# danavery/audio-tokens

Hardware: AMD Instinct MI355X
Metric: STFT frames/sec through K-means+tokenize, n_mels=64 vocab=8192 (higher is better)
Workload: dtype f32; 1 GPU; configs[3] per-GPU shard x1: 22500+2500 clips/GPU of 10 s @22.05 kHz (43075000 frames/GPU), n_mels=64, vocab_size=8192, niter=20, k-means batches of 10000 files on a 2097152-row subsample; parallelism=dp1

## Files before the change

audio_tokens_amd/_lib.py:

```python
from __future__ import annotations

import ctypes
from pathlib import Path

_PKG = Path(__file__).resolve().parent
LIB_PATH = _PKG / "libaudio_tokens_amd.so"

AT_LAYOUT_MEL_MAJOR = 0
AT_LAYOUT_FRAME_MAJOR = 1

_c = ctypes
_vp, _i32, _i64 = _c.c_void_p, _c.c_int, _c.c_int64

class PrunedArgs(_c.Structure):
    _fields_ = [("x", _vp), ("n", _i64), ("d", _i32), ("c", _vp), ("k", _i32), ("order", _vp), ("hint_sorted", _vp),
                ("cperm", _vp), ("ng", _i32), ("bounds", _vp), ("guess_only", _i32), ("use_filter", _i32),
                ("prepass_done", _i32), ("image_current", _i32), ("ids", _vp), ("dist_or_null", _vp)]


class FlacInfo(_c.Structure):
    _fields_ = [("channels", _c.c_int32), ("bits_per_sample", _c.c_int32), ("sample_rate", _c.c_int32),
                ("min_block", _c.c_int32), ("max_block", _c.c_int32), ("variable_blocksize", _c.c_int32),
                ("total_samples", _i64)]

# ... 25 lines not shown
    "at_workspace_bytes": (_i64, [_vp]),
    "at_background_stream": (_i32, [_vp, _c.POINTER(_vp)]),
    "at_debug_set": (_i32, [_vp, _c.c_char_p, _i32]),
    "at_debug_get": (_i32, [_vp, _c.c_char_p, _c.POINTER(_i32)]),
    "at_diag_errors": (_i32, [_c.POINTER(_i64), _c.POINTER(_i32), _c.POINTER(_i64), _c.POINTER(_i32), _c.c_char_p, _i32, _i32]),
    "at_debug_leave_error_pending": (_i32, []),
    "at_rand_perm_mt19937": (_i32, [_i64, _i64, _vp]),
    "at_rand_perm_prefix_mt19937": (_i32, [_i64, _i64, _i64, _vp]),
    "at_rand_perm_prefix_device": (_i32, [_vp, _i64, _i64, _i64, _vp, _vp]),
    "at_mel_filterbank_host": (_i32, [_i32, _i32, _i32, _vp]),
    "at_num_frames": (_i64, [_i64, _i32]),
    "at_split_clusters_host": (_i32, [_i32, _i32, _i64, _vp, _vp, _c.POINTER(_i32)]),
    "at_logmel_f32": (_i32, [_vp, _vp, _i64, _i64, _i64, _i32, _i32, _i32, _i32, _vp, _vp, _i32, _i32, _vp]),
    "at_resample_length": (_i64, [_i64, _i32, _i32]),
    "at_resample_taps_host": (_i32, [_i32, _i32, _c.POINTER(_i32), _c.POINTER(_i32), _c.POINTER(_i32), _vp, _i64]),
    "at_resample_f32": (_i32, [_vp, _vp, _i64, _i64, _i64, _i32, _i32, _vp, _i64, _vp]),
    "at_minmax_scale_clips_f32": (_i32, [_vp, _vp, _i64, _i64, _vp]),
    "at_conv1d_mel_f32": (_i32, [_vp, _vp, _i64, _i32, _vp, _vp, _i32, _i32, _i32, _vp, _vp]),
    "at_logmel_minmax_f32": (_i32, [_vp, _vp, _i64, _i64, _i64, _i32, _i32, _i32, _i32, _vp, _vp, _i32, _vp]),
    "at_l2norm_rows_f32": (_i32, [_vp, _vp, _i64, _i32, _vp, _vp]),
    "at_assign_f32": (_i32, [_vp, _vp, _i64, _i32, _vp, _i32, _vp, _vp, _vp]),
    "at_assign_hinted_f32": (_i32, [_vp, _vp, _i64, _i32, _vp, _i32, _vp, _vp, _vp, _vp, _vp, _vp]),
    "at_group_rows_kd_host": (_i32, [_vp, _i32, _i32, _i32, _vp]),
    "at_group_min_dist_f32": (_i32, [_vp, _vp, _i32, _i32, _vp, _i32, _vp, _vp]),
    "at_visit_order_f32": (_i32, [_vp, _vp, _vp, _i64, _i32, _vp, _vp, _vp]),
    "at_prune_stats": (_i32, [_vp, _c.POINTER(_i64), _c.POINTER(_i64), _i32]),
    "at_assign_coarse_f32": (_i32, [_vp, _vp, _i64, _i32, _vp, _i32, _vp, _i32, _vp, _vp, _vp, _vp, _vp]),
    "at_filter_stats": (_i32, [_vp, _c.POINTER(_i64), _c.POINTER(_i64), _c.POINTER(_c.c_double), _c.POINTER(_i64),
                               _c.POINTER(_i64), _c.POINTER(_i64), _i32]),
    "at_filter_probe_f32": (_i32, [_vp, _vp, _i64, _i32, _vp, _i32, _vp, _vp, _vp, _i32, _vp, _vp, _vp,
                                   _c.POINTER(_i64), _vp]),
    "at_group_means_f32": (_i32, [_vp, _vp, _i32, _i32, _vp, _i32, _vp, _vp]),
    "at_group_neighbours_f32": (_i32, [_vp, _vp, _i32, _i32, _i32, _vp, _vp]),
    "at_assign_pruned_f32": (_i32, [_vp, _vp, _vp]),
    "at_prune_mask_f32": (_i32, [_vp, _vp, _i64, _i32, _vp, _i32, _vp, _vp, _i32, _vp, _i32, _vp]),
    "at_gather_rows_f32": (_i32, [_vp, _vp, _i32, _vp, _i64, _vp, _vp]),
    "at_centroid_accum_f32": (_i32, [_vp, _vp, _i64, _i32, _vp, _i32, _vp, _vp, _vp, _vp, _vp]),
    "at_centroid_finalize_f32": (_i32, [_vp, _vp, _i64, _vp, _i64, _i32, _i32, _i32, _vp, _vp, _vp]),
    "at_split_clusters_f32": (_i32, [_vp, _i32, _i32, _i64, _vp, _vp, _vp, _vp]),
    "at_lloyd_stats_f64": (_i32, [_vp, _vp, _i32, _vp, _i64, _i32, _vp, _vp]),
    "at_comm_allgather_f32": (_i32, [_vp, _vp, _vp, _vp, _i64, _vp]),
    "at_comm_allreduce_ordered_f32": (_i32, [_vp, _vp, _vp, _vp, _vp, _i64, _vp]),
    "at_lloyd_stats_split_f32": (_i32, [_vp, _i32, _i32, _i64, _vp, _vp, _vp, _vp, _i64, _i32, _vp, _vp]),
    "at_sum_parts_f32": (_i32, [_vp, _vp, _i64, _i32, _i64, _vp, _vp]),
    "at_sum_f32": (_i32, [_vp, _vp, _i64, _vp, _vp]),
    "at_any_nonfinite_f32": (_i32, [_vp, _vp, _i64, _vp, _vp]),
    "at_logmel_nonfinite_take": (_i32, [_vp, _vp, _vp]),
    "at_centroid_accum_defer": (_i32, [_vp, _i32]),
    "at_centroid_accum_join": (_i32, [_vp, _vp]),
    "at_token_histogram_i64": (_i32, [_vp, _vp, _i64, _i32, _vp, _vp]),
    "at_token_stats_f64": (_i32, [_vp, _vp, _i32, _vp, _vp, _vp, _vp]),
    "at_silhouette_f32": (_i32, [_vp, _vp, _i32, _vp, _i64, _vp, _vp, _vp, _vp]),
    "at_average_precision_f32": (_i32, [_vp, _vp, _i64, _vp, _i64, _i64, _i32, _vp, _vp, _vp, _vp, _vp]),
    "at_ranking_metrics_f32": (_i32, [_vp, _vp, _i64, _vp, _i64, _i64, _i32, _vp, _vp, _vp, _vp, _vp, _vp, _vp, _vp]),
    "at_threshold_counts_f32": (_i32, [_vp, _vp, _i64, _vp, _i64, _i64, _i32, _c.c_float, _vp, _vp, _vp]),
    "at_knn_f32": (_i32, [_vp, _vp, _i64, _i32, _vp, _i32, _i32, _vp, _vp, _vp]),
    "at_assign_ip_f32": (_i32, [_vp, _vp, _i64, _i32, _vp, _i32, _vp, _vp, _vp]),
    "at_renorm_rows_f32": (_i32, [_vp, _vp, _i64, _i32, _vp]),
    "at_pq_encode_f32": (_i32, [_vp, _vp, _i64, _i32, _i32, _i32, _vp, _vp, _vp, _vp, _vp]),
    "at_pq_decode_f32": (_i32, [_vp, _vp, _i64, _i32, _i32, _i32, _vp, _vp, _vp]),
    "at_flac_index_host": (_i32, [_vp, _i64, _c.POINTER(FlacInfo), _vp, _i64, _c.POINTER(_i64)]),
    "at_flac_decode_f32": (_i32, [_vp, _i64, _vp, _i64, _i32, _vp, _i64, _vp, _vp, _vp]),
# ... 79 lines not shown
```

audio_tokens_amd/backend.py:

```python
from __future__ import annotations

import ctypes
import os

import numpy as np
import torch

from . import _lib

_vp = ctypes.c_void_p


def _ptr(t) -> _vp:
    return _vp(t.data_ptr()) if t is not None else _vp(None)


def _np_ptr(a: np.ndarray) -> _vp:
    return _vp(a.ctypes.data)


class HostHelpers:

    def __init__(self):
        self.lib = _lib.load()
# ... 107 lines not shown
        return int(ns.value)


class HipBackend(HostHelpers):
    def __init__(self, device=None):
        super().__init__()
        if not torch.cuda.is_available():
            raise RuntimeError("audio_tokens_amd: no ROCm device visible (torch.cuda.is_available() "
                               "is False) and there is no CPU fallback")
        if device is None:
            device = torch.device("cuda", torch.cuda.current_device())
        device = torch.device(device)
        if device.type != "cuda":
            raise RuntimeError(f"audio_tokens_amd: device must be a ROCm GPU, got {device}")
        if device.index is None:
            device = torch.device("cuda", torch.cuda.current_device())
        self.device = device
        self.ctx = _lib.context(device.index)
        self.assign_trace = None
        self.assign_trace_only = None
        self.frontend_calls = 0
        self.frontend_bytes = 0
        self.switches = {"filter": os.environ.get("AT_FILTER", "1") != "0",
                         "c2f_fused": os.environ.get("AT_C2F_FUSED", "1") != "0"}

    def debug_set(self, name: str, value: int) -> None:
        _lib.check(self.lib.at_debug_set(self.ctx.handle, name.encode(), int(value)))

    def debug_get(self, name: str) -> int:
        v = ctypes.c_int(0)
        _lib.check(self.lib.at_debug_get(self.ctx.handle, name.encode(), ctypes.byref(v)))
        return int(v.value)

    def diag_errors(self, reset=False) -> dict:
        stale, tol = ctypes.c_int64(0), ctypes.c_int64(0)
        sc, tc = ctypes.c_int(0), ctypes.c_int(0)
        where = ctypes.create_string_buffer(512)
        _lib.check(self.lib.at_diag_errors(ctypes.byref(stale), ctypes.byref(sc), ctypes.byref(tol), ctypes.byref(tc),
                                           where, 512, 1 if reset else 0))
        return {"stale_seen": int(stale.value), "stale_last_code": int(sc.value), "tolerated": int(tol.value),
                "tolerated_last_code": int(tc.value), "where": where.value.decode()}

    def _stream(self) -> _vp:
        return _vp(torch.cuda.current_stream(self.device).cuda_stream)

    def _f32(self, t, name="tensor") -> torch.Tensor:
        if isinstance(t, np.ndarray):
# ... 405 lines not shown
        if rec is not None:
            e0, e1 = torch.cuda.Event(enable_timing=True), torch.cuda.Event(enable_timing=True)
            e0.record(torch.cuda.current_stream(self.device))
        with torch.cuda.device(self.device):
            _lib.check(self.lib.at_assign_hinted_f32(self.ctx.handle, _ptr(x), n, d, _ptr(c), k, _ptr(hint_ids),
                                                     _ptr(order), _ptr(hint_sorted), _ptr(ids), _ptr(dist),
                                                     self._stream()))
        if rec is not None:
            e1.record(torch.cuda.current_stream(self.device))
            rec.append(("hinted", n, d, k, e0, e1))
        return ids, dist

    def group_min_dist(self, c, cperm) -> torch.Tensor:
        c = self._f32(c)
        k, d = c.shape
        assert cperm.dtype == torch.int32 and cperm.is_contiguous() and cperm.numel() % 32 == 0
        ng = cperm.numel() // 32
        dmin = self.empty((k, ng))
        with torch.cuda.device(self.device):
            _lib.check(self.lib.at_group_min_dist_f32(self.ctx.handle, _ptr(c), k, d, _ptr(cperm), ng, _ptr(dmin),
                                                      self._stream()))
        return dmin

    def visit_order(self, ids, dis, k):
        n = ids.numel()
        assert ids.dtype == torch.int64 and ids.is_contiguous()
        order, hs = self.empty((n,), torch.int32), self.empty((n,), torch.int32)
        with torch.cuda.device(self.device):
            _lib.check(self.lib.at_visit_order_f32(self.ctx.handle, _ptr(ids), _ptr(dis), n, k, _ptr(order), _ptr(hs),
                                                   self._stream()))
        return order, hs

    def visit_order_beside(self, ids, dis, k, sum_out=None):
        main = torch.cuda.current_stream(self.device)
        side = getattr(self, "_order_stream", None)
        if side is None:
            side = self._order_stream = torch.cuda.Stream(self.device)
        side.wait_stream(main)
        with torch.cuda.stream(side):
            if sum_out is not None:
                self.sum_f64(dis, out=sum_out)
                sum_out.record_stream(side)
            out = self.visit_order(ids, dis, k)

        def join(out=out, ids=ids, dis=dis):
            torch.cuda.current_stream(self.device).wait_stream(side)
# ... 199 lines not shown

    def centroid_finalize(self, parts, k, d):
        if parts.dim() == 1:
            parts = parts.unsqueeze(0)
        assert parts.is_contiguous() and parts.shape[1] >= k * d + k
        n_parts = parts.shape[0]
        cent = self.empty((k, d))
        hassign = self.empty((k,))
        stride = parts.stride(0)
        with torch.cuda.device(self.device):
            _lib.check(self.lib.at_centroid_finalize_f32(
                self.ctx.handle, _ptr(parts), stride, _vp(parts.data_ptr() + 4 * k * d), stride, n_parts,
                k, d, _ptr(cent), _ptr(hassign), self._stream()))
        return cent, hassign

    def split_clusters_device(self, hassign, cent, n: int, nsplit_out) -> None:
        k, d = cent.shape
        assert hassign.dtype == torch.float32 and cent.dtype == torch.float32 and nsplit_out.dtype == torch.int32
        assert hassign.is_contiguous() and cent.is_contiguous() and hassign.numel() == k
        with torch.cuda.device(self.device):
            _lib.check(self.lib.at_split_clusters_f32(self.ctx.handle, d, k, n, _ptr(hassign), _ptr(cent), _ptr(nsplit_out),
                                                      self._stream()))

    def _objective_parts(self, parts, k, d, objs):
        if objs is not None:
            assert objs.dtype == torch.float64 and objs.is_contiguous()
            return _ptr(objs), 1, objs.numel()
        if parts.dim() == 1:
            parts = parts.unsqueeze(0)
        off, total = self.part_layout(k, d)
        assert parts.is_contiguous() and parts.shape[1] == total
        return _vp(parts.data_ptr() + 4 * off), total // 2, parts.shape[0]

    def lloyd_stats(self, hassign, parts, k: int, d: int, stats_row, objs=None) -> None:
        assert stats_row.dtype == torch.float64
        ptr, stride, n_parts = self._objective_parts(parts, k, d, objs)
        with torch.cuda.device(self.device):
            _lib.check(self.lib.at_lloyd_stats_f64(self.ctx.handle, _ptr(hassign), k, ptr, stride, n_parts, _ptr(stats_row),
                                                   self._stream()))

    def lloyd_stats_split(self, hassign, cent, n: int, nsplit_out, parts, stats_row, objs=None) -> None:
        k, d = cent.shape
        assert stats_row.dtype == torch.float64 and nsplit_out.dtype == torch.int32
        assert hassign.dtype == torch.float32 and cent.dtype == torch.float32
        assert hassign.is_contiguous() and cent.is_contiguous() and hassign.numel() == k
        ptr, stride, n_parts = self._objective_parts(parts, k, d, objs)
# ... 144 lines not shown
```

audio_tokens_amd/csrc/lloyd.hip:

```cpp
#include <climits>

#include "at_internal.h"
#include "mt19937_dev.h"

namespace {

constexpr int WG = 256;
constexpr long SPLIT_CYCLES = 64;
constexpr int SPLIT_BLOCKS = 16;
constexpr int SPLIT_ROUND = SPLIT_BLOCKS * WG;

__device__ __forceinline__ float rand_float_of(uint32_t raw) { return __uint2float_rn(raw) * 2.3283064365386963e-10f; }

__device__ void lloyd_stats_block(const float* __restrict__ hassign, int k, const double* obj_parts, long obj_stride,
                                  int n_parts, double* __restrict__ stats) {
    __shared__ double s1[WG / 64], s2[WG / 64];
    const int t = threadIdx.x;
    double a = 0.0, b = 0.0;
    for (int c = t; c < k; c += WG) {
        const double h = (double)hassign[c];
        a += h;
        b += h * h;
    }
    for (int off = 32; off > 0; off >>= 1) {
        a += __shfl_down(a, off);
        b += __shfl_down(b, off);
    }
    if ((t & 63) == 0) { s1[t >> 6] = a; s2[t >> 6] = b; }
    __syncthreads();
    if (t == 0) {
        double tot = 0.0, sq = 0.0;
        for (int w = 0; w < WG / 64; w++) { tot += s1[w]; sq += s2[w]; }
        double obj = 0.0;
        for (int p = 0; p < n_parts; p++) obj += obj_parts[(size_t)p * obj_stride];
        stats[0] = obj;
        stats[1] = sq * k / (tot * tot);
    }
    __syncthreads();
}

__global__ __launch_bounds__(WG) void lloyd_stats_kernel(const float* __restrict__ hassign, int k, const double* obj_parts,
                                                        long obj_stride, int n_parts, double* __restrict__ stats) {
    lloyd_stats_block(hassign, k, obj_parts, obj_stride, n_parts, stats);
}

__global__ __launch_bounds__(WG) void split_clusters_kernel(int d, int k, long n, float* hassign, float* cent,
                                                           int* __restrict__ empties, int* __restrict__ nsplit_out,
                                                           const uint32_t* __restrict__ raw, long raw_n,
                                                           const uint32_t* __restrict__ state_end, int p_lds,
                                                           const double* obj_parts, long obj_stride, int n_parts,
                                                           double* __restrict__ stats) {
    extern __shared__ float pl[];
    __shared__ at_mt::State mt;
    __shared__ float draws[at_mt::N];
    __shared__ int wave_val[4][WG / 64];
    __shared__ int n_empty;
    const int t = threadIdx.x, lane = t & 63, wave = t >> 6;

    if (stats) lloyd_stats_block(hassign, k, obj_parts, obj_stride, n_parts, stats);
    {
        bool any = false;
        for (int c = t; c < k; c += WG) any |= hassign[c] == 0.0f;
        if (!__syncthreads_or(any)) {
            if (t == 0) *nsplit_out = 0;
            return;
        }
    }
    if (t == 0) n_empty = 0;
    __syncthreads();
    for (int base = 0; base < k; base += WG) {
        const int c = base + t;
        const bool e = c < k && hassign[c] == 0.0f;
        const unsigned long long b = __ballot(e);
        if (lane == 0) wave_val[0][wave] = __popcll(b);
        __syncthreads();
        int off = n_empty;
        for (int w = 0; w < wave; w++) off += wave_val[0][w];
        if (e) empties[off + __popcll(b & ((1ull << lane) - 1ull))] = c;
        __syncthreads();
        if (t == 0) n_empty += wave_val[0][0] + wave_val[0][1] + wave_val[0][2] + wave_val[0][3];
        __syncthreads();
    }
    const int ne = n_empty;
    if (ne == 0) {
        if (t == 0) *nsplit_out = 0;
        return;
    }

    const double denom = (double)(float)(n - k);
    auto prob = [&](int c) { return (float)(((double)hassign[c] - 1.0) / denom); };
    if (p_lds) {
        for (int c = t; c < k; c += WG) pl[c] = prob(c);
        __syncthreads();
    }
    const double up = 1.0 + 1.0 / 1024.0, down = 1.0 - 1.0 / 1024.0;
    long pos = 0;
    int cur = 0, win = 0, wlen = 0;
    bool own = false;
    int done = 0;
    for (int e = 0; e < ne; e++) {
        const int ci = empties[e];
        int cj0 = 0, donor = -1;
        long left = SPLIT_CYCLES * k + 1024;
        while (left > 0 && donor < 0) {
            if (pos + SPLIT_ROUND <= raw_n) {
                uint32_t draw[SPLIT_BLOCKS];
#pragma unroll
                for (int i = 0; i < SPLIT_BLOCKS; i++) draw[i] = raw[pos + i * WG + t];
                int mine = INT_MAX;
#pragma unroll
                for (int i = 0; i < SPLIT_BLOCKS; i++) {
                    const int j = i * WG + t;
                    int cj = cj0 + j;
                    cj -= (cj / k) * k;
                    const float pc = p_lds ? pl[cj] : prob(cj);
                    const bool acc = rand_float_of(draw[i]) < pc;
                    const unsigned long long b = __ballot(acc);
                    if (b && mine == INT_MAX) mine = i * WG + wave * 64 + (__ffsll((long long)b) - 1);
                }
                if (lane == 0) wave_val[0][wave] = mine;
                __syncthreads();
                int first = INT_MAX;
#pragma unroll
                for (int w = 0; w < WG / 64; w++) first = min(first, wave_val[0][w]);
                __syncthreads();
                if (first != INT_MAX) {
                    donor = (int)((cj0 + (long)first) % k);
                    pos += first + 1;
                } else {
                    pos += SPLIT_ROUND;
                    left -= SPLIT_ROUND;
                    cj0 = (int)((cj0 + (long)SPLIT_ROUND) % k);
                }
                continue;
            }
            if (win == wlen) {
                if (pos < raw_n) {
                    wlen = (int)min((long)at_mt::N, raw_n - pos);
                    for (int q = t; q < wlen; q += WG) draws[q] = rand_float_of(raw[pos + q]);
                } else {
                    wlen = at_mt::N;
                    if (!own) {
                        for (int q = t; q < at_mt::N; q += WG) mt.st[0][q] = state_end[q];
                        __syncthreads();
                        own = true;
                        cur = 0;
                    }
                    const uint32_t* nw = at_mt::regenerate(mt, cur);
// ... 8 lines not shown
            if (t < chunk) {
                const int cj = (cj0 + t) % k;
                acc = draws[win + t] < (p_lds ? pl[cj] : prob(cj));
            }
            const unsigned long long b = __ballot(acc);
            if (lane == 0) wave_val[0][wave] = b ? wave * 64 + (__ffsll((long long)b) - 1) : INT_MAX;
            __syncthreads();
            const int first = min(min(wave_val[0][0], wave_val[0][1]), min(wave_val[0][2], wave_val[0][3]));
            __syncthreads();
            if (first < chunk) {
                donor = (cj0 + first) % k;
                win += first + 1;
                pos += first + 1;
            } else {
                win += chunk;
                pos += chunk;
                left -= chunk;
                cj0 = (cj0 + chunk) % k;
            }
        }
        if (donor < 0) break;
        float* dst = cent + (size_t)ci * d;
        float* src = cent + (size_t)donor * d;
        for (int j = t; j < d; j += WG) {
            const double a = (double)src[j];
            dst[j] = (float)(a * ((j & 1) ? down : up));
            src[j] = (float)(a * ((j & 1) ? up : down));
        }
        if (t == 0) {
            const float half = hassign[donor] / 2;
            hassign[ci] = half;
            hassign[donor] -= half;
        }
        done++;
        __syncthreads();
        if (p_lds && t == 0) {
            pl[ci] = prob(ci);
            pl[donor] = prob(donor);
        }
        __syncthreads();
    }
    if (t == 0) *nsplit_out = done == ne ? ne : -1;
}

}

extern "C" {

int at_split_clusters_f32(at_ctx* ctx, int d, int k, int64_t n, float* hassign, float* centroids, int32_t* nsplit_out,
                          void* stream_) {
    return at_lloyd_stats_split_f32(ctx, d, k, n, hassign, centroids, nsplit_out, nullptr, 0, 0, nullptr, stream_);
}

int at_lloyd_stats_split_f32(at_ctx* ctx, int d, int k, int64_t n, float* hassign, float* centroids, int32_t* nsplit_out,
                             const double* obj_parts, int64_t obj_part_stride, int n_parts, double* stats, void* stream_) {
    AT_REQUIRE(ctx && hassign && centroids && nsplit_out && d > 0 && k > 0 && n >= k, "at_split_clusters_f32: bad arguments");
    AT_REQUIRE(!stats || (obj_parts && n_parts >= 1 && (reinterpret_cast<uintptr_t>(obj_parts) & 7u) == 0 &&
                          (reinterpret_cast<uintptr_t>(stats) & 7u) == 0),
               "at_lloyd_stats_split_f32: obj_parts / stats must be given together, 8-byte aligned");
    hipStream_t stream = static_cast<hipStream_t>(stream_);
    AT_HIP(hipSetDevice(ctx->device));
    int* empties = static_cast<int*>(at_ws(ctx, WS_SPLIT_LIST, (size_t)k * sizeof(int), stream));
    if (!empties) return AT_E_NOMEM;
    const uint32_t *raw = nullptr, *state_end = nullptr;
    int64_t raw_n = 0;
    int rc = at_mt_cached_draws(ctx, 1234u, stream, &raw, &raw_n, &state_end);
    if (rc) return rc;
    const int p_lds = k <= 16384;
    const size_t lds = p_lds ? (size_t)k * sizeof(float) : 0;
    AT_RAISE_LDS(ctx, split_clusters_kernel, lds);
    AT_LAUNCH(split_clusters_kernel, dim3(1), dim3(WG), lds, stream, d, k, (long)n, hassign, centroids, empties,
                       nsplit_out, raw, (long)raw_n, state_end, p_lds, obj_parts, (long)obj_part_stride, n_parts, stats);
    return AT_OK;
}

int at_lloyd_stats_f64(at_ctx* ctx, const float* hassign, int k, const double* obj_parts, int64_t obj_part_stride,
                       int n_parts, double* stats, void* stream_) {
    AT_REQUIRE(ctx && hassign && obj_parts && stats && k > 0 && n_parts >= 1, "at_lloyd_stats_f64: bad arguments");
    AT_REQUIRE((reinterpret_cast<uintptr_t>(obj_parts) & 7u) == 0 && (reinterpret_cast<uintptr_t>(stats) & 7u) == 0,
               "at_lloyd_stats_f64: obj_parts / stats must be 8-byte aligned");
    hipStream_t stream = static_cast<hipStream_t>(stream_);
    AT_HIP(hipSetDevice(ctx->device));
    AT_LAUNCH(lloyd_stats_kernel, dim3(1), dim3(WG), 0, stream, hassign, k, obj_parts, (long)obj_part_stride,
                       n_parts, stats);
    return AT_OK;
}

}
```

audio_tokens_amd/ops.py:

```python
from __future__ import annotations

import collections
import math
import os
import statistics
import sys
import time
from collections import OrderedDict

import numpy as np
import torch

from .backend import default_backend

__all__ = ["LogMelSpectrogram", "Resample", "Kmeans", "IndexFlatL2", "IndexFlatIP", "normalize_rows", "silhouette_samples",
           "silhouette_score", "average_precision", "mean_average_precision", "roc_auc", "mean_roc_auc",
           "roc_auc_score", "d_prime", "f1_score", "hamming_loss", "classification_metrics", "load_flac",
           "load_flac_batch", "AudioTokenizer", "ProductQuantizer"]


def _is_host(x) -> bool:
    return isinstance(x, np.ndarray) or (isinstance(x, torch.Tensor) and x.device.type == "cpu")


# ... 267 lines not shown

        niter = self.niter
        stats_dev = be.zeros((max(niter, 1), 2), torch.float64)
        nsplit_dev = be.zeros((max(niter, 1),), torch.int32)
        obj_off, part_len = be.part_layout(k, d)
        scatter_exchange = dist.on and (self.exchange == "scatter" or (self.exchange == "auto" and part_len * 4 > (4 << 20)))
        t0 = time.time()
        prof = self.phase_seconds

        def lap(name, t_prev):
            if prof is None:
                return t_prev
            be.synchronize()
            now = time.perf_counter()
            prof[name] = prof.get(name, 0.0) + (now - t_prev)
            return now

        prune = (self.prune and not spherical and hasattr(be, "assign_pruned") and d in (64, 128) and k >= 1024
                 and (k + 31) // 32 <= 512 and xs.shape[0] >= 4096)
        ids = dis = order = vorder = None
        member_order = prune and xs.shape[0] < 96 * k
        regrouping = None
        regrouping_is_late = False

        def regroup_beside(c):
            h, ready = be.to_host_async(c)

            def job():
                ready.synchronize()
                return be.group_rows_kd(h.numpy())
            return _grouper().submit(job)

        if prune:
            upload = getattr(be, "from_host_async", be.from_host)
            cached = getattr(self, "_cperm_cache", None)
            if init_centroids is not None and cached is not None and cached[0] == (k, d):
                cperm = cached[1]
                if not (init_centroids is getattr(self, "centroids_device", None)
                        or init_centroids is self.__dict__.get("_centroids_host")):
                    regrouping = regroup_beside(cent)
            else:
                cperm = be.from_host(be.group_rows_kd(be.to_host(cent)))
            gnbr = None
        late_regroup = niter - 6 if niter >= 10 else -1
        paced = collections.deque()
        iter_ms = None
        last_done = None
        timed_events = hasattr(be, "record_event_timed")

        def late_due(it):
            if late_regroup < 0 or it < niter // 2:
                return False
            return it >= late_regroup or (iter_ms is not None and (niter - it) * iter_ms <= 4.5)

        def pruned_assign(it):
            nonlocal cperm, regrouping, regrouping_is_late, gnbr
            if regrouping is not None and regrouping.done():
                cperm = upload(regrouping.result())
                regrouping = None
            elif (it == 2 and init_centroids is None and regrouping is None) or (late_due(it) and not regrouping_is_late):
                regrouping_is_late = late_due(it)
                regrouping = regroup_beside(cent)
            dmin = be.group_min_dist(cent, cperm)
            if ids is None:
                gnbr = be.group_neighbours(be.group_means(cent, cperm), 8)
                return be.assign_c2f(xs, cent, cperm, dmin, gnbr)
            return be.assign_pruned(xs, cent, vorder if vorder is not None else be.visit_order(ids, dis, k),
                                    cperm, dmin, image_current=True)

        for it in range(niter):
            tp = time.perf_counter()
            if prune:
                ids, dis = pruned_assign(it)
            elif spherical:
                ids, dis = be.assign_ip(xs, cent)
            elif ids is None:
                ids, dis = be.assign(xs, cent)
            else:
                ids, dis = be.assign_hinted(xs, cent, ids, order)
            tp = lap("assign", tp)
            part = be.empty((part_len,))
            obj_view = part[obj_off:obj_off + 2].view(torch.float64)
            beside = prune and not member_order and self.order_beside and it + 1 < niter
            sjoin = None
            if not beside:
# ... 30 lines not shown
            if hasattr(be, "lloyd_stats_split"):
                be.lloyd_stats_split(hassign, cent, ns, nsplit_dev[it:it + 1], parts, stats_dev[it], objs=objs)
            else:
                be.lloyd_stats(hassign, parts, k, d, stats_dev[it], objs=objs)
                be.split_clusters_device(hassign, cent, ns, nsplit_dev[it:it + 1])
            if spherical:
                cent = be.renorm_rows(cent)
            tp = lap("exchange+finalize+split", tp)
            if prune and timed_events:
                paced.append(be.record_event_timed())
                if len(paced) > 3:
                    done = paced.popleft()
                    done.synchronize()
                    if last_done is not None:
                        iter_ms = last_done.elapsed_time(done)
                    last_done = done
        self._last_assign = ids
        self._stats_pending = (stats_dev[:niter], nsplit_dev[:niter], t0)
        if self.verbose:
            for it, st in enumerate(self.iteration_stats):
                print(f"  Iteration {it} ({st['time']:.2f} s, search {st['time_search']:.2f} s): "
                      f"objective={st['obj']:g} imbalance={st['imbalance_factor']:.3f} nsplit={st['nsplit']}", flush=True)
        if prune:
            if regrouping is not None and (regrouping.done() or regrouping_is_late):
                cperm = upload(regrouping.result())
            self._cperm_cache = ((k, d), cperm)
            self._grouping_of_result = cperm
        return self._finish(cent, sync)

    def _subsample_perm(self, n, m):
        key = (int(n), self.seed, int(m))
        cache = self.__dict__.setdefault("_perm_cache", OrderedDict())
        hit = cache.get(key)
        if hit is None:
            hit = cache[key] = self.backend.rand_perm_prefix_device(n, self.seed, m)
            while len(cache) > 2:
                cache.popitem(last=False)
        return hit

    def _read_stats(self, stats_dev, nsplit_dev, t0):
        be = self.backend
        st, ns = be.to_host(stats_dev), be.to_host(nsplit_dev)
        if (ns < 0).any():
            raise RuntimeError("Kmeans: split_clusters found no donor (every cluster has at most one point)")
        el = time.time() - t0
        return [dict(obj=float(np.float32(st[i, 0])), time=el * (i + 1) / len(ns), time_search=el * (i + 1) / len(ns),
                     imbalance_factor=float(st[i, 1]), nsplit=int(ns[i])) for i in range(len(ns))]

    @property
    def iteration_stats(self):
        if self._stats_pending is not None:
            self._iteration_stats = self._read_stats(*self._stats_pending)
            self._stats_pending = None
        return self._iteration_stats

    @property
    def obj(self):
        return np.array([s["obj"] for s in self.iteration_stats], dtype=np.float32)

    @property
    def centroids(self):
        if self._centroids_host is None and self.centroids_device is not None:
            self._centroids_host = self.backend.to_host(self.centroids_device)
        return self._centroids_host

    def lend_grouping(self, table) -> None:
        cached = getattr(self, "_cperm_cache", None)
        be = self.backend
        if cached is not None and hasattr(be, "remember_grouping"):
            table = be.to_host(table) if isinstance(table, torch.Tensor) else np.asarray(table)
            if table.shape == cached[0]:
                be.remember_grouping(table, cached[1])

    def _finish(self, cent, sync=True):
        self.centroids_device = cent
        self._centroids_host = None
        self.index = (IndexFlatIP if self.spherical else IndexFlatL2)(self.d, backend=self.backend)
        self.index.add(cent)
        be = self.backend
        if getattr(self, "_grouping_of_result", None) is not None and hasattr(be, "remember_grouping"):
            if sync:
                be.remember_grouping(self.centroids, self._grouping_of_result)
            self._grouping_of_result = None
        if not sync:
            return None
        st = self.iteration_stats
        return float(st[-1]["obj"]) if st else 0.0


_GROUPER = None


def _grouper():
    global _GROUPER
    if _GROUPER is None:
        from concurrent.futures import ThreadPoolExecutor
        _GROUPER = ThreadPoolExecutor(max_workers=1, thread_name_prefix="at-grouping")
    return _GROUPER


class IndexFlatL2:

    def __init__(self, d, backend=None):
        self.d = int(d)
        self.backend = backend or default_backend()
        self._c = None
        self._prune = None
        self.prune = True
        self.rows_coherent = True

    @property
    def ntotal(self) -> int:
        return 0 if self._c is None else int(self._c.shape[0])

    def reset(self) -> None:
        self._c = None
        self._prune = None

    def add(self, c) -> None:
        c = self.backend._f32(c)
        assert c.dim() == 2 and c.shape[1] == self.d, f"expected [n, {self.d}]"
        self._c = c.clone() if self._c is None else torch.cat([self._c, c], 0)
        self._prune = None

    def assign(self, x, want_dist=True):
        be = self.backend
        c = self._c
        k = c.shape[0]
        if (self.prune and hasattr(be, "assign_c2f") and self.d in (64, 128) and k >= 1024
                and (k + 31) // 32 <= 512 and x.shape[0] >= 65536):
            if self._prune is None:
                c_host = be.to_host(c)
                cperm = be.recall_grouping(c_host) if hasattr(be, "recall_grouping") else None
                if cperm is None or cperm.numel() != ((k + 31) // 32) * 32:
                    cperm = be.from_host(be.group_rows_kd(c_host))
                self._prune = (cperm, be.group_min_dist(c, cperm), be.group_neighbours(be.group_means(c, cperm), 4))
            cperm, dmin, gnbr = self._prune
            return be.assign_c2f(x, c, cperm, dmin, gnbr, want_dist=want_dist, coherent=self.rows_coherent)
        if (self.prune and hasattr(be, "assign_unguided") and self.d in (64, 128) and 128 <= k < 1024 and x.shape[0] >= 65536
                and getattr(be, "switches", {}).get("filter", True)):
            if self._prune is None:
                self._prune = (be.from_host(be.group_rows_kd(be.to_host(c))), None, None)
            return be.assign_unguided(x, c, want_dist=want_dist, cperm=self._prune[0])
        return be.assign(x, c, want_dist=want_dist)

    def search(self, x, k=1):
        if k < 1:
            raise RuntimeError(f"IndexFlatL2.search: k must be at least 1, got {k}")
        if k != 1:
            return self._search_k(x, int(k))
        host = _is_host(x)
        be = self.backend
        x = be._f32(x)
        assert x.dim() == 2 and x.shape[1] == self.d, f"expected [n, {self.d}]"
        if self._c is None:
            D = torch.full((x.shape[0], 1), float("inf"), device=be.device)
            I = torch.full((x.shape[0], 1), -1, dtype=torch.int64, device=be.device)
        else:
            ids, dis = self.assign(x)
            D, I = dis.unsqueeze(1), ids.unsqueeze(1)
        return (be.to_host(D), be.to_host(I)) if host else (D, I)

    def _search_k(self, x, k):
        be = self.backend
        if not hasattr(be, "knn"):
# ... 354 lines not shown
```

include/audio_tokens_amd.h:

```cpp
#ifndef AUDIO_TOKENS_AMD_H
#define AUDIO_TOKENS_AMD_H

#include <stdint.h>

#ifdef __cplusplus
extern "C" {
#endif

#define AT_VERSION 100

#define AT_OK 0
#define AT_E_INVALID (-1)
#define AT_E_HIP (-2)
#define AT_E_NOMEM (-3)
#define AT_E_TOO_FEW (-4)
#define AT_E_NONFINITE (-5)
#define AT_E_COMM (-6)

#define AT_LAYOUT_MEL_MAJOR 0
#define AT_LAYOUT_FRAME_MAJOR 1

typedef struct at_ctx at_ctx;

int at_version(void);
// ... 71 lines not shown
                          at_frontend_totals* totals);

int at_mix_resample_ragged_f32(at_ctx* ctx, const float* in, const at_frontend_clip* plan_dev, const int32_t* order_dev,
                               const at_frontend_group* group, float* mono, void* stream);

int at_logmel_ragged_f32(at_ctx* ctx, const float* mono, const at_frontend_clip* plan_dev, int64_t n_clips,
                         const at_frontend_totals* totals, int sample_rate, int n_fft, int hop, int n_mels,
                         const float* fb_or_null, float* out, int layout, int fuse_l2norm, int32_t* bad, void* stream);

int at_logmel_ragged_minmax_f32(at_ctx* ctx, const float* mono, const at_frontend_clip* plan_dev, int64_t n_clips,
                                const at_frontend_totals* totals, int sample_rate, int n_fft, int hop, int n_mels,
                                const float* fb_or_null, float* out, int layout, int fuse_l2norm, int32_t* bad,
                                void* stream);

int at_assign_f32(at_ctx* ctx, const float* x, int64_t n, int d, const float* c, int k,
                  int64_t* ids, float* dist_or_null, void* stream);

int at_assign_hinted_f32(at_ctx* ctx, const float* x, int64_t n, int d, const float* c, int k,
                         const int64_t* hint_ids_or_null, const uint32_t* order_or_null,
                         const uint32_t* hint_sorted_or_null, int64_t* ids, float* dist_or_null,
                         void* stream);

int at_group_rows_kd_host(const float* rows_host, int k, int d, int leaf, int32_t* perm_out_host);
int at_group_min_dist_f32(at_ctx* ctx, const float* c, int k, int d, const int32_t* cperm, int ng,
                          float* dmin, void* stream);
int at_visit_order_f32(at_ctx* ctx, const int64_t* ids, const float* dis_or_null, int64_t n, int k,
                       uint32_t* order_out, uint32_t* hint_sorted_out, void* stream);
int at_group_means_f32(at_ctx* ctx, const float* c, int k, int d, const int32_t* cperm, int ng,
                       float* means, void* stream);
int at_group_neighbours_f32(at_ctx* ctx, const float* means, int ng, int d, int nnb, uint32_t* gnbr,
                            void* stream);
typedef struct at_pruned_args {
    const float* x;
    int64_t n;
    int d;
    const float* c;
    int k;
    const uint32_t* order;
    const uint32_t* hint_sorted;
    const int32_t* cperm;
    int ng;
    const float* bounds;
    int guess_only;
    int use_filter;
    int prepass_done;
    int image_current;
// ... 16 lines not shown
                       float* out, void* stream);

int at_centroid_accum_f32(at_ctx* ctx, const float* x, int64_t n, int d, const int64_t* ids, int k,
                          float* sums, float* counts, uint32_t* order_out_or_null,
                          uint32_t* sorted_ids_out_or_null, void* stream);

int at_centroid_accum_defer(at_ctx* ctx, int on);
int at_centroid_accum_join(at_ctx* ctx, void* stream);

int at_centroid_finalize_f32(at_ctx* ctx, const float* sums_parts, int64_t sums_part_stride,
                             const float* counts_parts, int64_t counts_part_stride, int n_parts,
                             int k, int d, float* centroids, float* hassign, void* stream);

int at_sum_parts_f32(at_ctx* ctx, const float* parts, int64_t part_stride, int n_parts, int64_t m, float* out,
                     void* stream);

int at_comm_allgather_f32(at_ctx* ctx, void* nccl_comm, const float* part, float* parts, int64_t count, void* stream);
int at_comm_allreduce_ordered_f32(at_ctx* ctx, void* nccl_comm, const float* part, float* parts_scratch, float* out,
                                  int64_t count, void* stream);

int at_split_clusters_f32(at_ctx* ctx, int d, int k, int64_t n, float* hassign, float* centroids,
                          int32_t* nsplit_out, void* stream);

int at_lloyd_stats_f64(at_ctx* ctx, const float* hassign, int k, const double* obj_parts,
                       int64_t obj_part_stride, int n_parts, double* stats, void* stream);

int at_lloyd_stats_split_f32(at_ctx* ctx, int d, int k, int64_t n, float* hassign, float* centroids, int32_t* nsplit_out,
                             const double* obj_parts, int64_t obj_part_stride, int n_parts, double* stats, void* stream);

int at_sum_f32(at_ctx* ctx, const float* v, int64_t n, double* out, void* stream);

int at_any_nonfinite_f32(at_ctx* ctx, const float* v, int64_t n, int32_t* flag, void* stream);

int at_logmel_nonfinite_take(at_ctx* ctx, int32_t* flag, void* stream);

int at_token_histogram_i64(at_ctx* ctx, const int64_t* ids, int64_t n, int k, int64_t* counts, void* stream);

int at_token_stats_f64(at_ctx* ctx, const int64_t* counts, int k, int64_t* sorted_counts,
                       int32_t* sorted_tokens, double* stats, void* stream);

int at_silhouette_f32(at_ctx* ctx, const float* x, int d, const int64_t* labels, int64_t n, float* s,
                      double* sum, int64_t* n_labels, void* stream);

int at_average_precision_f32(at_ctx* ctx, const float* scores, int64_t ld_scores, const float* labels, int64_t ld_labels,
                             int64_t n, int c, double* ap, int64_t* n_pos, double* map, int32_t* flags, void* stream);

// ... 66 lines not shown
```

Baseline: 279.1 million frames/s.

## Build centroid k-d grouping on the GPU and window split-cluster draws in LDS

Adds a GPU kernel that recursively bisects the centroids by a power-iteration principal axis and bitonic-sorts the projections. It replaces the host k-d grouping and its device-host round trips, is on by default, can run on a side stream, and has an optional regroup-every-iteration mode. Separately, the split-clusters kernel now stages random draws into an LDS window as floats using vectorised loads and steps the candidate index incrementally. This grouping may differ from the host version and change how well pruning works.

Result: no change. 278.8 million frames/s (-0.1%).

```diff
diff --git a/audio_tokens_amd/_lib.py b/audio_tokens_amd/_lib.py
--- a/audio_tokens_amd/_lib.py
+++ b/audio_tokens_amd/_lib.py
@@ -71,6 +71,7 @@
     "at_assign_f32": (_i32, [_vp, _vp, _i64, _i32, _vp, _i32, _vp, _vp, _vp]),
     "at_assign_hinted_f32": (_i32, [_vp, _vp, _i64, _i32, _vp, _i32, _vp, _vp, _vp, _vp, _vp, _vp]),
     "at_group_rows_kd_host": (_i32, [_vp, _i32, _i32, _i32, _vp]),
+    "at_group_rows_kd_f32": (_i32, [_vp, _vp, _i32, _i32, _i32, _vp, _vp]),
     "at_group_min_dist_f32": (_i32, [_vp, _vp, _i32, _i32, _vp, _i32, _vp, _vp]),
     "at_visit_order_f32": (_i32, [_vp, _vp, _vp, _i64, _i32, _vp, _vp, _vp]),
     "at_prune_stats": (_i32, [_vp, _c.POINTER(_i64), _c.POINTER(_i64), _i32]),
@@ -87,6 +88,7 @@
     "at_centroid_accum_f32": (_i32, [_vp, _vp, _i64, _i32, _vp, _i32, _vp, _vp, _vp, _vp, _vp]),
     "at_centroid_finalize_f32": (_i32, [_vp, _vp, _i64, _vp, _i64, _i32, _i32, _i32, _vp, _vp, _vp]),
     "at_split_clusters_f32": (_i32, [_vp, _i32, _i32, _i64, _vp, _vp, _vp, _vp]),
+    "at_split_window_draws": (_i32, []),
     "at_lloyd_stats_f64": (_i32, [_vp, _vp, _i32, _vp, _i64, _i32, _vp, _vp]),
     "at_comm_allgather_f32": (_i32, [_vp, _vp, _vp, _vp, _i64, _vp]),
     "at_comm_allreduce_ordered_f32": (_i32, [_vp, _vp, _vp, _vp, _vp, _i64, _vp]),
diff --git a/audio_tokens_amd/backend.py b/audio_tokens_amd/backend.py
--- a/audio_tokens_amd/backend.py
+++ b/audio_tokens_amd/backend.py
@@ -153,7 +153,9 @@
         self.frontend_calls = 0
         self.frontend_bytes = 0
         self.switches = {"filter": os.environ.get("AT_FILTER", "1") != "0",
-                         "c2f_fused": os.environ.get("AT_C2F_FUSED", "1") != "0"}
+                         "c2f_fused": os.environ.get("AT_C2F_FUSED", "1") != "0",
+                         "device_grouping": os.environ.get("AT_DEVICE_GROUPING", "1") != "0",
+                         "regroup_every": os.environ.get("AT_REGROUP_EVERY", "0") != "0"}
 
     def debug_set(self, name: str, value: int) -> None:
         _lib.check(self.lib.at_debug_set(self.ctx.handle, name.encode(), int(value)))
@@ -605,6 +607,33 @@
                                                       self._stream()))
         return dmin
 
+    def group_rows_kd_device(self, c, leaf: int = 32) -> torch.Tensor:
+        c = self._f32(c)
+        k, d = c.shape
+        out = torch.empty((((k + leaf - 1) // leaf) * leaf,), dtype=torch.int32, device=self.device)
+        with torch.cuda.device(self.device):
+            _lib.check(self.lib.at_group_rows_kd_f32(self.ctx.handle, _ptr(c), k, d, int(leaf), _ptr(out), self._stream()))
+        return out
+
+    def group_rows_kd_beside(self, c, leaf: int = 32):
+        main = torch.cuda.current_stream(self.device)
+        side = getattr(self, "_order_stream", None)
+        if side is None:
+            side = self._order_stream = torch.cuda.Stream(self.device)
+        side.wait_stream(main)
+        with torch.cuda.stream(side):
+            out = self.group_rows_kd_device(c, leaf)
+            c.record_stream(side)
+            ready = torch.cuda.Event()
+            ready.record(side)
+
+        def join(out=out, c=c):
+            cur = torch.cuda.current_stream(self.device)
+            cur.wait_event(ready)
+            out.record_stream(cur)
+            return out
+        return join
+
     def visit_order(self, ids, dis, k):
         n = ids.numel()
         assert ids.dtype == torch.int64 and ids.is_contiguous()
@@ -850,6 +879,9 @@
             _lib.check(self.lib.at_split_clusters_f32(self.ctx.handle, d, k, n, _ptr(hassign), _ptr(cent), _ptr(nsplit_out),
                                                       self._stream()))
 
+    def split_window_draws(self) -> int:
+        return int(self.lib.at_split_window_draws())
+
     def _objective_parts(self, parts, k, d, objs):
         if objs is not None:
             assert objs.dtype == torch.float64 and objs.is_contiguous()
diff --git a/audio_tokens_amd/csrc/group.hip b/audio_tokens_amd/csrc/group.hip
--- /dev/null
+++ b/audio_tokens_amd/csrc/group.hip
@@ -0,0 +1,207 @@
+#include <algorithm>
+
+#include "at_internal.h"
+
+namespace {
+
+constexpr int GROUP_MAX_ROWS = 16384;
+constexpr int GROUP_MAX_D = 256;
+constexpr int LPR = 16;
+
+__device__ __forceinline__ float sum16(float v) {
+    v += __shfl_xor(v, 8);
+    v += __shfl_xor(v, 4);
+    v += __shfl_xor(v, 2);
+    v += __shfl_xor(v, 1);
+    return v;
+}
+
+__device__ __forceinline__ float dot_lds(const float* a, const float* b, int d) {
+    float s = 0.0f;
+    for (int f = 0; f < d; f++) s = __builtin_fmaf(a[f], b[f], s);
+    return s;
+}
+
+__device__ __forceinline__ uint32_t float_key(float v) {
+    const uint32_t u = __float_as_uint(v + 0.0f);
+    return (u & 0x80000000u) ? ~u : (u | 0x80000000u);
+}
+
+__global__ __launch_bounds__(256) void group_init_kernel(int k, int n_out, int32_t* __restrict__ idx) {
+    const int i = blockIdx.x * blockDim.x + threadIdx.x;
+    if (i < n_out) idx[i] = i < k ? i : -1;
+}
+
+enum { PASS_MEAN = 0, PASS_POWER = 1, PASS_PROJECT = 2 };
+
+template <int J, int PASS>
+__device__ void group_pass(const float* __restrict__ rows, int d, const int32_t* part, int m, const float* mean,
+                           const float* axis, float* scratch, float* out, unsigned long long* keys) {
+    const int t = threadIdx.x, l = t & (LPR - 1), slot = t / LPR, slots = blockDim.x / LPR;
+    float4 mu[J], ax[J], acc[J];
+#pragma unroll
+    for (int j = 0; j < J; j++) {
+        const int f = 4 * (l + LPR * j);
+        const bool in = f < d;
+        mu[j] = PASS != PASS_MEAN && in ? *reinterpret_cast<const float4*>(mean + f) : make_float4(0.f, 0.f, 0.f, 0.f);
+        ax[j] = PASS != PASS_MEAN && in ? *reinterpret_cast<const float4*>(axis + f) : make_float4(0.f, 0.f, 0.f, 0.f);
+        acc[j] = make_float4(0.f, 0.f, 0.f, 0.f);
+    }
+    constexpr int U = 8 / J;
+    for (int i0 = 0; i0 < m; i0 += slots * U) {
+        int row[U];
+        bool live[U];
+#pragma unroll
+        for (int u = 0; u < U; u++) {
+            const int i = i0 + u * slots + slot;
+            live[u] = i < m;
+            row[u] = live[u] ? part[i] : 0;
+        }
+        float4 c[U][J];
+#pragma unroll
+        for (int u = 0; u < U; u++) {
+            const float* r = rows + (size_t)row[u] * d;
+#pragma unroll
+            for (int j = 0; j < J; j++) {
+                const int f = 4 * (l + LPR * j);
+                c[u][j] = live[u] && f < d ? *reinterpret_cast<const float4*>(r + f) : make_float4(0.f, 0.f, 0.f, 0.f);
+            }
+        }
+#pragma unroll
+        for (int u = 0; u < U; u++) {
+            if (PASS == PASS_MEAN) {
+#pragma unroll
+                for (int j = 0; j < J; j++) {
+                    acc[j].x += c[u][j].x; acc[j].y += c[u][j].y; acc[j].z += c[u][j].z; acc[j].w += c[u][j].w;
+                }
+                continue;
+            }
+            float dot = 0.0f;
+#pragma unroll
+            for (int j = 0; j < J; j++) {
+                float4& v = c[u][j];
+                v.x -= mu[j].x; v.y -= mu[j].y; v.z -= mu[j].z; v.w -= mu[j].w;
+                dot = __builtin_fmaf(v.x, ax[j].x, dot);
+                dot = __builtin_fmaf(v.y, ax[j].y, dot);
+                dot = __builtin_fmaf(v.z, ax[j].z, dot);
+                dot = __builtin_fmaf(v.w, ax[j].w, dot);
+            }
+            dot = sum16(dot);
+            if (PASS == PASS_POWER) {
+                if (live[u]) {
+#pragma unroll
+                    for (int j = 0; j < J; j++) {
+                        acc[j].x = __builtin_fmaf(dot, c[u][j].x, acc[j].x);
+                        acc[j].y = __builtin_fmaf(dot, c[u][j].y, acc[j].y);
+                        acc[j].z = __builtin_fmaf(dot, c[u][j].z, acc[j].z);
+                        acc[j].w = __builtin_fmaf(dot, c[u][j].w, acc[j].w);
+                    }
+                }
+            } else if (live[u] && l == 0) {
+                keys[i0 + u * slots + slot] = ((unsigned long long)float_key(dot) << 32) | (uint32_t)row[u];
+            }
+        }
+    }
+    if (PASS == PASS_PROJECT) return;
+#pragma unroll
+    for (int j = 0; j < J; j++) {
+        const int f = 4 * (l + LPR * j);
+        if (f < d) *reinterpret_cast<float4*>(scratch + (size_t)slot * d + f) = acc[j];
+    }
+    __syncthreads();
+    for (int f = t; f < d; f += blockDim.x) {
+        float s = 0.0f;
+        for (int q = 0; q < slots; q++) s += scratch[(size_t)q * d + f];
+        out[f] = s;
+    }
+    __syncthreads();
+}
+
+template <int J>
+__global__ __launch_bounds__(1024) void group_level_kernel(const float* __restrict__ rows, int k, int d, int leaf, int ng,
+                                                          int level, int key_cap, int32_t* idx) {
+    extern __shared__ __attribute__((aligned(16))) unsigned char smem[];
+    unsigned long long* keys = reinterpret_cast<unsigned long long*>(smem);
+    float* scratch = reinterpret_cast<float*>(smem);
+    __shared__ __attribute__((aligned(16))) float mean[GROUP_MAX_D], axis[GROUP_MAX_D], next[GROUP_MAX_D];
+    const int t = threadIdx.x, T = blockDim.x;
+    int g0 = 0, g1 = ng;
+    for (int b = level - 1; b >= 0; b--) {
+        if (g1 - g0 <= 1) return;
+        const int gmid = g0 + (g1 - g0) / 2;
+        if ((blockIdx.x >> b) & 1) g0 = gmid; else g1 = gmid;
+    }
+    if (g1 - g0 <= 1) return;
+    const int lo = g0 * leaf, hi = min(g1 * leaf, k), m = hi - lo;
+    int n2 = 1;
+    while (n2 < m) n2 <<= 1;
+    if (m <= 0 || n2 > key_cap) return;
+    int32_t* part = idx + lo;
+
+    group_pass<J, PASS_MEAN>(rows, d, part, m, nullptr, nullptr, scratch, mean, nullptr);
+    for (int f = t; f < d; f += T) {
+        mean[f] = mean[f] / (float)m;
+        axis[f] = 1.0f + 0.01f * (float)f;
+    }
+    __syncthreads();
+    for (int it = 0; it < 4; it++) {
+        group_pass<J, PASS_POWER>(rows, d, part, m, mean, axis, scratch, next, nullptr);
+        const float nrm = dot_lds(next, next, d);
+        if (!(nrm > 0.0f)) break;
+        const float inv = 1.0f / __builtin_sqrtf(nrm);
+        for (int f = t; f < d; f += T) axis[f] = next[f] * inv;
+        __syncthreads();
+    }
+    group_pass<J, PASS_PROJECT>(rows, d, part, m, mean, axis, nullptr, nullptr, keys);
+    for (int i = m + t; i < n2; i += T) keys[i] = ~0ull;
+    __syncthreads();
+    for (int size = 2; size <= n2; size <<= 1) {
+        for (int stride = size >> 1; stride > 0; stride >>= 1) {
+            for (int i = t; i < n2 / 2; i += T) {
+                const int a = 2 * i - (i & (stride - 1)), b = a + stride;
+                const unsigned long long ka = keys[a], kb = keys[b];
+                const bool up = (a & size) == 0;
+                if ((ka > kb) == up) {
+                    keys[a] = kb;
+                    keys[b] = ka;
+                }
+            }
+            __syncthreads();
+        }
+    }
+    for (int i = t; i < m; i += T) part[i] = (int32_t)(uint32_t)keys[i];
+}
+
+template <int J>
+int group_levels(at_ctx* ctx, const float* rows, int k, int d, int leaf, int ng, int32_t* idx, hipStream_t stream) {
+    int nlevels = 0;
+    while ((1 << nlevels) < ng) nlevels++;
+    for (int level = 0; level < nlevels; level++) {
+        const int gmax = (ng + (1 << level) - 1) >> level;
+        const int mmax = (int)std::min<int64_t>((int64_t)gmax * leaf, k);
+        int n2 = 1;
+        while (n2 < mmax) n2 <<= 1;
+        const int threads = mmax > 2048 ? 1024 : 256;
+        const size_t lds = std::max((size_t)n2 * 8, (size_t)(threads / LPR) * d * sizeof(float));
+        AT_RAISE_LDS(ctx, group_level_kernel<J>, lds);
+        AT_LAUNCH(group_level_kernel<J>, dim3(1u << level), dim3(threads), lds, stream, rows, k, d, leaf, ng, level, n2, idx);
+    }
+    return AT_OK;
+}
+
+}
+
+extern "C" int at_group_rows_kd_f32(at_ctx* ctx, const float* rows, int k, int d, int leaf, int32_t* perm_out, void* stream_) {
+    AT_REQUIRE(ctx && rows && perm_out && k > 0 && d > 0 && leaf > 0, "at_group_rows_kd_f32: bad arguments");
+    AT_REQUIRE(k <= GROUP_MAX_ROWS && leaf <= GROUP_MAX_ROWS && d <= GROUP_MAX_D && d % 4 == 0 && (reinterpret_cast<uintptr_t>(rows) & 15u) == 0,
+               "at_group_rows_kd_f32: at most %d rows of at most %d features, d a multiple of 4, rows 16-byte aligned (k=%d d=%d)",
+               GROUP_MAX_ROWS, GROUP_MAX_D, k, d);
+    hipStream_t stream = static_cast<hipStream_t>(stream_);
+    AT_HIP(hipSetDevice(ctx->device));
+    const int ng = (k + leaf - 1) / leaf;
+    const int n_out = ng * leaf;
+    AT_LAUNCH(group_init_kernel, dim3((n_out + 255) / 256), dim3(256), 0, stream, k, n_out, perm_out);
+    if (d <= 64) return group_levels<1>(ctx, rows, k, d, leaf, ng, perm_out, stream);
+    if (d <= 128) return group_levels<2>(ctx, rows, k, d, leaf, ng, perm_out, stream);
+    return group_levels<4>(ctx, rows, k, d, leaf, ng, perm_out, stream);
+}
diff --git a/audio_tokens_amd/csrc/lloyd.hip b/audio_tokens_amd/csrc/lloyd.hip
--- a/audio_tokens_amd/csrc/lloyd.hip
+++ b/audio_tokens_amd/csrc/lloyd.hip
@@ -9,6 +9,10 @@
 constexpr long SPLIT_CYCLES = 64;
 constexpr int SPLIT_BLOCKS = 16;
 constexpr int SPLIT_ROUND = SPLIT_BLOCKS * WG;
+constexpr int SPLIT_WINDOW = 16384;
+constexpr int SPLIT_FILL_LOADS = SPLIT_WINDOW / 4 / WG;
+static_assert(SPLIT_WINDOW % (4 * WG) == 0 && SPLIT_WINDOW - 3 >= SPLIT_ROUND, "a window holds a whole step from any position");
+static_assert(AT_MT_CACHE_DRAWS % 4 == 0, "the resident stream ends on a 16-byte boundary");
 
 __device__ __forceinline__ float rand_float_of(uint32_t raw) { return __uint2float_rn(raw) * 2.3283064365386963e-10f; }
 
@@ -50,7 +54,8 @@
                                                            const uint32_t* __restrict__ state_end, int p_lds,
                                                            const double* obj_parts, long obj_stride, int n_parts,
                                                            double* __restrict__ stats) {
-    extern __shared__ float pl[];
+    extern __shared__ __attribute__((aligned(16))) float pl[];
+    float* const window = pl + (p_lds ? (k + 3) & ~3 : 0);
     __shared__ at_mt::State mt;
     __shared__ float draws[at_mt::N];
     __shared__ int wave_val[4][WG / 64];
@@ -93,37 +98,60 @@
         for (int c = t; c < k; c += WG) pl[c] = prob(c);
         __syncthreads();
     }
+    auto prob_of = [&](float h) { return (float)(((double)h - 1.0) / denom); };
     const double up = 1.0 + 1.0 / 1024.0, down = 1.0 - 1.0 / 1024.0;
     long pos = 0;
+    long wbase = 0;
+    int wfill = 0, par = 0;
+    const long raw_fast = raw_n & ~3L;
+    const int wg_step = WG % k;
     int cur = 0, win = 0, wlen = 0;
     bool own = false;
     int done = 0;
+    int ci_next = empties[0];
     for (int e = 0; e < ne; e++) {
-        const int ci = empties[e];
+        const int ci = ci_next;
+        if (e + 1 < ne) ci_next = empties[e + 1];
         int cj0 = 0, donor = -1;
         long left = SPLIT_CYCLES * k + 1024;
         while (left > 0 && donor < 0) {
-            if (pos + SPLIT_ROUND <= raw_n) {
-                uint32_t draw[SPLIT_BLOCKS];
-#pragma unroll
-                for (int i = 0; i < SPLIT_BLOCKS; i++) draw[i] = raw[pos + i * WG + t];
+            if (pos + SPLIT_ROUND <= raw_fast) {
+                if (pos + SPLIT_ROUND > wbase + wfill) {
+                    wbase = pos & ~3L;
+                    wfill = (int)min((long)SPLIT_WINDOW, raw_fast - wbase);
+                    const uint4* src4 = reinterpret_cast<const uint4*>(raw + wbase);
+                    const int qlast = wfill / 4 - 1;
+                    uint4 v[SPLIT_FILL_LOADS];
+#pragma unroll
+                    for (int i = 0; i < SPLIT_FILL_LOADS; i++) v[i] = src4[min(i * WG + t, qlast)];
+                    __builtin_amdgcn_sched_barrier(0);
+#pragma unroll
+                    for (int i = 0; i < SPLIT_FILL_LOADS; i++) {
+                        const int q = i * WG + t;
+                        reinterpret_cast<float4*>(window)[q] = make_float4(rand_float_of(v[i].x), rand_float_of(v[i].y),
+                                                                           rand_float_of(v[i].z), rand_float_of(v[i].w));
+                    }
+                    __syncthreads();
+                }
+                const float* wd = window + (int)(pos - wbase) + t;
+                int cj = cj0 + t;
+                cj -= (cj / k) * k;
                 int mine = INT_MAX;
 #pragma unroll
                 for (int i = 0; i < SPLIT_BLOCKS; i++) {
-                    const int j = i * WG + t;
-                    int cj = cj0 + j;
-                    cj -= (cj / k) * k;
                     const float pc = p_lds ? pl[cj] : prob(cj);
-                    const bool acc = rand_float_of(draw[i]) < pc;
+                    const bool acc = wd[i * WG] < pc;
                     const unsigned long long b = __ballot(acc);
                     if (b && mine == INT_MAX) mine = i * WG + wave * 64 + (__ffsll((long long)b) - 1);
-                }
-                if (lane == 0) wave_val[0][wave] = mine;
+                    cj += wg_step;
+                    if (cj >= k) cj -= k;
+                }
+                if (lane == 0) wave_val[2 + par][wave] = mine;
                 __syncthreads();
                 int first = INT_MAX;
 #pragma unroll
-                for (int w = 0; w < WG / 64; w++) first = min(first, wave_val[0][w]);
-                __syncthreads();
+                for (int w = 0; w < WG / 64; w++) first = min(first, wave_val[2 + par][w]);
+                par ^= 1;
                 if (first != INT_MAX) {
                     donor = (int)((cj0 + (long)first) % k);
                     pos += first + 1;
@@ -178,22 +206,22 @@
         if (donor < 0) break;
         float* dst = cent + (size_t)ci * d;
         float* src = cent + (size_t)donor * d;
+        const float hd = t == 0 ? hassign[donor] : 0.0f;
         for (int j = t; j < d; j += WG) {
             const double a = (double)src[j];
             dst[j] = (float)(a * ((j & 1) ? down : up));
             src[j] = (float)(a * ((j & 1) ? up : down));
         }
         if (t == 0) {
-            const float half = hassign[donor] / 2;
+            const float half = hd / 2, rest = hd - half;
             hassign[ci] = half;
-            hassign[donor] -= half;
+            hassign[donor] = rest;
+            if (p_lds) {
+                pl[ci] = prob_of(half);
+                pl[donor] = prob_of(rest);
+            }
         }
         done++;
-        __syncthreads();
-        if (p_lds && t == 0) {
-            pl[ci] = prob(ci);
-            pl[donor] = prob(donor);
-        }
         __syncthreads();
     }
     if (t == 0) *nsplit_out = done == ne ? ne : -1;
@@ -223,12 +251,14 @@
     int rc = at_mt_cached_draws(ctx, 1234u, stream, &raw, &raw_n, &state_end);
     if (rc) return rc;
     const int p_lds = k <= 16384;
-    const size_t lds = p_lds ? (size_t)k * sizeof(float) : 0;
+    const size_t lds = ((p_lds ? ((size_t)k + 3) & ~(size_t)3 : 0) + SPLIT_WINDOW) * sizeof(float);
     AT_RAISE_LDS(ctx, split_clusters_kernel, lds);
     AT_LAUNCH(split_clusters_kernel, dim3(1), dim3(WG), lds, stream, d, k, (long)n, hassign, centroids, empties,
                        nsplit_out, raw, (long)raw_n, state_end, p_lds, obj_parts, (long)obj_part_stride, n_parts, stats);
     return AT_OK;
 }
+
+int at_split_window_draws(void) { return SPLIT_WINDOW; }
 
 int at_lloyd_stats_f64(at_ctx* ctx, const float* hassign, int k, const double* obj_parts, int64_t obj_part_stride,
                        int n_parts, double* stats, void* stream_) {
diff --git a/audio_tokens_amd/ops.py b/audio_tokens_amd/ops.py
--- a/audio_tokens_amd/ops.py
+++ b/audio_tokens_amd/ops.py
@@ -313,8 +313,13 @@
         member_order = prune and xs.shape[0] < 96 * k
         regrouping = None
         regrouping_is_late = False
+        regrouped_at = 0
+        dev_group = prune and _device_grouping(be)
+        regroup_every = dev_group and be.switches.get("regroup_every", False)
 
         def regroup_beside(c):
+            if dev_group:
+                return be.group_rows_kd_beside(c)
             h, ready = be.to_host_async(c)
 
             def job():
@@ -324,12 +329,20 @@
 
         if prune:
             upload = getattr(be, "from_host_async", be.from_host)
+
+            def arrived(job, it):
+                return it > regrouped_at if dev_group else job.done()
+
+            def taken(job):
+                return job() if dev_group else upload(job.result())
             cached = getattr(self, "_cperm_cache", None)
             if init_centroids is not None and cached is not None and cached[0] == (k, d):
                 cperm = cached[1]
                 if not (init_centroids is getattr(self, "centroids_device", None)
                         or init_centroids is self.__dict__.get("_centroids_host")):
                     regrouping = regroup_beside(cent)
+            elif dev_group:
+                cperm = be.group_rows_kd_device(cent)
             else:
                 cperm = be.from_host(be.group_rows_kd(be.to_host(cent)))
             gnbr = None
@@ -345,13 +358,17 @@
             return it >= late_regroup or (iter_ms is not None and (niter - it) * iter_ms <= 4.5)
 
         def pruned_assign(it):
-            nonlocal cperm, regrouping, regrouping_is_late, gnbr
-            if regrouping is not None and regrouping.done():
-                cperm = upload(regrouping.result())
+            nonlocal cperm, regrouping, regrouping_is_late, regrouped_at, gnbr
+            if regrouping is not None and arrived(regrouping, it):
+                cperm = taken(regrouping)
                 regrouping = None
+                if regroup_every and it + 1 < niter:
+                    regrouping, regrouped_at = regroup_beside(cent), it
+            elif regroup_every and regrouping is None and it >= 1 and it + 1 < niter:
+                regrouping, regrouped_at = regroup_beside(cent), it
             elif (it == 2 and init_centroids is None and regrouping is None) or (late_due(it) and not regrouping_is_late):
                 regrouping_is_late = late_due(it)
-                regrouping = regroup_beside(cent)
+                regrouping, regrouped_at = regroup_beside(cent), it
             dmin = be.group_min_dist(cent, cperm)
             if ids is None:
                 gnbr = be.group_neighbours(be.group_means(cent, cperm), 8)
@@ -428,8 +445,8 @@
                 print(f"  Iteration {it} ({st['time']:.2f} s, search {st['time_search']:.2f} s): "
                       f"objective={st['obj']:g} imbalance={st['imbalance_factor']:.3f} nsplit={st['nsplit']}", flush=True)
         if prune:
-            if regrouping is not None and (regrouping.done() or regrouping_is_late):
-                cperm = upload(regrouping.result())
+            if regrouping is not None and (arrived(regrouping, niter) or regrouping_is_late):
+                cperm = taken(regrouping)
             self._cperm_cache = ((k, d), cperm)
             self._grouping_of_result = cperm
         return self._finish(cent, sync)
@@ -473,6 +490,8 @@
     def lend_grouping(self, table) -> None:
         cached = getattr(self, "_cperm_cache", None)
         be = self.backend
+        if _device_grouping(be):
+            return
         if cached is not None and hasattr(be, "remember_grouping"):
             table = be.to_host(table) if isinstance(table, torch.Tensor) else np.asarray(table)
             if table.shape == cached[0]:
@@ -485,13 +504,17 @@
         self.index.add(cent)
         be = self.backend
         if getattr(self, "_grouping_of_result", None) is not None and hasattr(be, "remember_grouping"):
-            if sync:
+            if sync and not _device_grouping(be):
                 be.remember_grouping(self.centroids, self._grouping_of_result)
             self._grouping_of_result = None
         if not sync:
             return None
         st = self.iteration_stats
         return float(st[-1]["obj"]) if st else 0.0
+
+
+def _device_grouping(be) -> bool:
+    return hasattr(be, "group_rows_kd_device") and bool(getattr(be, "switches", {}).get("device_grouping", False))
 
 
 _GROUPER = None
@@ -536,17 +559,21 @@
         if (self.prune and hasattr(be, "assign_c2f") and self.d in (64, 128) and k >= 1024
                 and (k + 31) // 32 <= 512 and x.shape[0] >= 65536):
             if self._prune is None:
-                c_host = be.to_host(c)
-                cperm = be.recall_grouping(c_host) if hasattr(be, "recall_grouping") else None
-                if cperm is None or cperm.numel() != ((k + 31) // 32) * 32:
-                    cperm = be.from_host(be.group_rows_kd(c_host))
+                if _device_grouping(be):
+                    cperm = be.group_rows_kd_device(c)
+                else:
+                    c_host = be.to_host(c)
+                    cperm = be.recall_grouping(c_host) if hasattr(be, "recall_grouping") else None
+                    if cperm is None or cperm.numel() != ((k + 31) // 32) * 32:
+                        cperm = be.from_host(be.group_rows_kd(c_host))
                 self._prune = (cperm, be.group_min_dist(c, cperm), be.group_neighbours(be.group_means(c, cperm), 4))
             cperm, dmin, gnbr = self._prune
             return be.assign_c2f(x, c, cperm, dmin, gnbr, want_dist=want_dist, coherent=self.rows_coherent)
         if (self.prune and hasattr(be, "assign_unguided") and self.d in (64, 128) and 128 <= k < 1024 and x.shape[0] >= 65536
                 and getattr(be, "switches", {}).get("filter", True)):
             if self._prune is None:
-                self._prune = (be.from_host(be.group_rows_kd(be.to_host(c))), None, None)
+                cperm = be.group_rows_kd_device(c) if _device_grouping(be) else be.from_host(be.group_rows_kd(be.to_host(c)))
+                self._prune = (cperm, None, None)
             return be.assign_unguided(x, c, want_dist=want_dist, cperm=self._prune[0])
         return be.assign(x, c, want_dist=want_dist)
 
diff --git a/include/audio_tokens_amd.h b/include/audio_tokens_amd.h
--- a/include/audio_tokens_amd.h
+++ b/include/audio_tokens_amd.h
@@ -117,6 +117,7 @@
                          void* stream);
 
 int at_group_rows_kd_host(const float* rows_host, int k, int d, int leaf, int32_t* perm_out_host);
+int at_group_rows_kd_f32(at_ctx* ctx, const float* rows, int k, int d, int leaf, int32_t* perm_out, void* stream);
 int at_group_min_dist_f32(at_ctx* ctx, const float* c, int k, int d, const int32_t* cperm, int ng,
                           float* dmin, void* stream);
 int at_visit_order_f32(at_ctx* ctx, const int64_t* ids, const float* dis_or_null, int64_t n, int k,
@@ -179,6 +180,8 @@
 int at_split_clusters_f32(at_ctx* ctx, int d, int k, int64_t n, float* hassign, float* centroids,
                           int32_t* nsplit_out, void* stream);
 
+int at_split_window_draws(void);
+
 int at_lloyd_stats_f64(at_ctx* ctx, const float* hassign, int k, const double* obj_parts,
                        int64_t obj_part_stride, int n_parts, double* stats, void* stream);
 
```
